# ToKe79/nuts333

Hardware: NVIDIA B200
Metric: rendered messages/sec (colour+swear+ban) (higher is better)
Workload: dtype u8

## Files before the change

### nuts333_b200/csrc/nutsb_kernels.cuh

```cuda
#pragma once
#include "nutsb_common.cuh"


struct OpsView {
    i64 n;
    const u8  *text;
    const u64 *toff;
    const u8  *kind;
    const i32 *target;
    const i32 *except_user;
    const u8  *flags;
    const i32 *gate;
    const u8  *verdict;
};

struct PopView {
    i32 n_users, n_rooms, n_rooms_tot;
    const i32 *user_room;
    const i32 *user_cls;
    const i32 *user_slot;
    const i32 *slot_user;
    const u8  *slot_cf;
    const u8  *slot_lv;
    const i32 *room_slot_off;
// ... 419 lines not shown
    u32 run_begin, run_cnt;
};

__device__ __forceinline__ uint4 nutsb_run_pack(u64 dst, u64 src, u32 len)
{
#ifdef NUTSB_EXPERIMENT_ALIGN
    dst &= ~(u64)(NUTSB_EXPERIMENT_ALIGN - 1); len = (len + NUTSB_EXPERIMENT_ALIGN - 1) & ~(u32)(NUTSB_EXPERIMENT_ALIGN - 1);
#endif
    return make_uint4((u32)dst, (u32)(dst >> 32), (u32)src, (len & 0xffffffu) | ((u32)(src >> 32) << 24));
}
#define NUTSB_RUN_MAX_LEN 0xffffffu

struct SlotInfo {
    u64 so_u;
    u64 end;
    u64 base;
    u32 b0, nb_room;
    u32 e0, e1;
    u32 room; i32 k;
    u32 cf_lv;
    u32 pad_;
};

struct SlotInfoArgs {
    PopView pop; ClassPrefix cpx;
    const u32 *room_b_off, *ev_off; const u64 *sv_pre, *stream_off;
    SlotInfo *out;
};

__global__ void __launch_bounds__(128)
k_slot_info(SlotInfoArgs A)
{
    const u32 s = blockIdx.x * blockDim.x + threadIdx.x;
    if (s >= (u32)A.pop.n_users) return;
    const i32 u = A.pop.slot_user[s];
    SlotInfo si;
    si.room = (u32)A.pop.user_room[u]; si.k = A.pop.user_cls[u];
    si.b0 = A.room_b_off[si.room]; si.nb_room = A.room_b_off[si.room + 1] - si.b0;
    si.e0 = A.ev_off[s]; si.e1 = A.ev_off[s + 1];
    si.so_u = A.stream_off[u]; si.end = A.stream_off[u + 1];
    si.base = si.so_u - A.cpx.at(si.k, si.room, si.b0) - A.sv_pre[si.e0];
    si.cf_lv = (u32)A.pop.slot_cf[s] | ((u32)A.pop.slot_lv[s] << 8);
    si.pad_ = 0;
    A.out[s] = si;
}

struct PlanArgs {
    PopView pop; Geometry geo; ClassPrefix cpx;
    const u64 *stream_off;
    const u32 *ev_off, *sv_ukey; const i32 *sv_delta; const u64 *sv_pre;
    const u32 *bl_meta;
    u64 n_cells, off_base;
    u32 has_level;
    const SlotInfo *slots;
    u32 *run_cursor;
    uint4 *runs; ItemDesc *items;
    u64 *counters;
    u32 *status;
};

template <bool FILL>
__device__ __forceinline__ u32 nutsb_plan_cell(const PlanArgs &A, u32 room, u32 t, u32 ls, u64 r_out, u32 &deliv, u32 &first)
{
    const SlotInfo si = A.slots[(u32)A.pop.room_slot_off[room] + ls];
    const u32 b0 = si.b0, nb_room = si.nb_room;
    const u32 a0 = t * NUTSB_TILE_OPS;
    const u32 nb = nb_room - a0 < NUTSB_TILE_OPS ? nb_room - a0 : NUTSB_TILE_OPS;
// ... 167 lines not shown
        const u32 l2 = (u32)idx & 15;
        const bool is_tail = idx >= 16;
        const u32 at = is_tail ? toff + l2 : l2;
        if (l2 < (is_tail ? tail : head)) dst[at] = src[at];
    }
    if (nvec == 0) return;
    dst += head; src += head;
    const u32 sm = (u32)((size_t)src & 15);
    const uint4 *sa = (const uint4 *)(src - sm);
    const u32 bsh = (sm & 3) * 8;
    switch (sm >> 2) {
    case 0:  nutsb_copy_body<0, WIDTH>(dst, sa, nvec, bsh, idx); break;
    case 1:  nutsb_copy_body<1, WIDTH>(dst, sa, nvec, bsh, idx); break;
    case 2:  nutsb_copy_body<2, WIDTH>(dst, sa, nvec, bsh, idx); break;
    default: nutsb_copy_body<3, WIDTH>(dst, sa, nvec, bsh, idx); break;
    }
}
__device__ __forceinline__ void nutsb_warp_copy(u8 *dst, const u8 *src, u32 n, int lane) { nutsb_group_copy<32>(dst, src, n, lane); }

#define NUTSB_REN_ON_WIN    3072
#define NUTSB_REN_OFF_WIN   1536
#define NUTSB_REN_ON_ROUND  (32 * 28)
#define NUTSB_REN_OFF_ROUND (32 * 8)
#define NUTSB_FL_COLOUR     0x100u

__device__ __forceinline__ u32 nutsb_keep_mask(i32 wb, i32 lo, i32 hi)
{
    i32 dl = lo - wb; dl = dl < 0 ? 0 : dl;
    i32 dh = wb + 4 - hi; dh = dh < 0 ? 0 : dh;
    const u32 a = dl >= 4 ? 0u : 0xffffffffu << (8 * dl);
    const u32 b = dh >= 4 ? 0u : 0xffffffffu >> (8 * dh);
    return a & b;
}

#define NUTSB_FLAT_META(al, n, fl) ((u32)(al) | ((u32)(n) << 2) | ((u32)(fl) << 14))

template <bool BOTH, class Sink>
__device__ __forceinline__ void nutsb_flat_render(u32 cnt, u32 meta, u64 gw, u32 nw,
                                                  u8 *w_on, u8 *w_off, const u8 *tab, int lane, Sink &sink)
{
    u32 inc = nw;
    for (int d = 1; d < 32; d <<= 1) { const u32 t = __shfl_up_sync(NUTSB_FULL, inc, d); if (lane >= d) inc += t; }
    const u32 P = inc - nw;
    const u32 W = __shfl_sync(NUTSB_FULL, inc, 31);
    u32 fill_on = 0, fill_off = 0, qcount = 0;
    u32 carry_x = 0, carry_m = 0;

    for (u32 F = 0; F < W; F += 32) {
        const bool starts = (u32)lane < cnt && P >= F && P < F + 32;
        const u32 heads = __reduce_or_sync(NUTSB_FULL, starts ? 1u << (P - F) : 0u);
        u32 q = qcount + (u32)__popc(heads & (0xffffffffu >> (31 - lane))) - 1;
        qcount += (u32)__popc(heads);
        if (q >= cnt) q = cnt - 1;
        const u32 Pq = __shfl_sync(NUTSB_FULL, P, (int)q), mq = __shfl_sync(NUTSB_FULL, meta, (int)q);
        const u32 *gwq = (const u32 *)(size_t)__shfl_sync(NUTSB_FULL, gw, (int)q);
        const u32 alq = mq & 3u, nq = (mq >> 2) & 0xfffu, flq = mq >> 14;
        const u32 endq = alq + nq;
        u32 nwq = (endq + 3) >> 2; if (!nwq) nwq = 1;
// ... 184 lines not shown
        __syncthreads();
        for (u32 r = (u32)warp / NUTSB_FAN_GROUP; r < nr; r += NUTSB_FAN_THREADS / 32 / NUTSB_FAN_GROUP) {
            const uint4 run = s_run[r];
            const u64 so = (u64)run.z | ((u64)(run.w >> 24) << 32);
            const u32 len = run.w & 0xffffffu;
            u8 *dst = A.out + (((u64)run.y << 32) | run.x);
            const u8 *src;
            if (!staged) src = A.slab + so;
            else if (so >= A.off_base) src = s_off + a_off + (u32)(so - d.off_src);
            else src = s_on + a_on + (u32)(so - d.on_src);
            nutsb_group_copy<32 * NUTSB_FAN_GROUP>(dst, src, len, tid % (32 * NUTSB_FAN_GROUP));
        }
    }
}

__global__ void __launch_bounds__(NUTSB_FAN_THREADS, NUTSB_FAN_MINBLOCKS)
k_fanout(FanoutArgs A)
{
    NUTSB_DYN_SMEM(s_dyn);
    nutsb_fanout_block(A, blockIdx.x, s_dyn);
}

struct DirectArgs {
    OpsView ops; PopView pop; ClassPrefix cpx;
    const u32 *room_b_off, *ev_off;
    const u32 *sv_ukey, *sv_op; const u64 *sv_pre;
    const u64 *stream_off;
    const u32 *ev_slot_sorted;
    const i32 *sv_delta;
    u8 *out; i64 n_ev;
    u64 *n_deliveries;
    u32 *status;
    const u8 *slab; u64 off_base;
    u32 has_level;
    const SlotInfo *slots;
    const u64 *dpre;
};

#define NUTSB_DIRECT_THREADS 256

struct DirectSink {
    u8 *out; u64 p; u32 O, osz;
    u32 cnt, done, qf;
    __device__ __forceinline__ void on(const u8 *w, u32 nbytes, int lane)
    {
        const u32 end = done + nbytes;
        while (qf < cnt) {
            const u32 Oq = __shfl_sync(NUTSB_FULL, O, (int)qf), zq = __shfl_sync(NUTSB_FULL, osz, (int)qf);
            const u64 pq = __shfl_sync(NUTSB_FULL, p, (int)qf);
            if (Oq >= end && zq) break;
            const u32 x0 = Oq > done ? Oq : done, x1 = Oq + zq < end ? Oq + zq : end;
            if (x1 > x0) {
                u8 *dst = out + pq + (x0 - Oq);
                const u8 *src = w + (x0 - done);
                const u32 len = x1 - x0;
                if (len < 192) { for (u32 i = (u32)lane; i < len; i += 32) dst[i] = src[i]; }
                else nutsb_warp_copy(dst, src, len, lane);
            }
            if (Oq + zq <= end) ++qf; else break;
        }
        done = end;
    }
    __device__ __forceinline__ void off(const u8 *, u32, int) {}
};

#define NUTSB_DIR_WARPS (NUTSB_DIRECT_THREADS / 32)
#define NUTSB_DIR_SMEM  (NUTSB_DIR_WARPS * (NUTSB_REN_ON_WIN + 64) + NUTSB_DIR_WARPS * 32 * (8 + 8 + 8) + ((NUTSB_CODETAB_BYTES + 15) & ~15))

template <bool COMPACT>
__device__ __forceinline__ void nutsb_direct_block(const DirectArgs &A, u32 blk, u32 nblk, u8 *smem)
{
    typedef u8 OnWin[NUTSB_REN_ON_WIN + 64];
    OnWin *const s_on = (OnWin *)smem;
    u64 (*const s_gw)[32] = (u64 (*)[32])(smem + NUTSB_DIR_WARPS * (NUTSB_REN_ON_WIN + 64));
    u64 (*const s_p)[32] = s_gw + NUTSB_DIR_WARPS;
    u32 (*const s_par)[32][2] = (u32 (*)[32][2])(s_p + NUTSB_DIR_WARPS);
    u8 *const s_tab = (u8 *)(s_par + NUTSB_DIR_WARPS);
    const int tid = threadIdx.x, lane = tid & 31, warp = tid >> 5;
    for (int i = tid; i < NUTSB_CODETAB_BYTES; i += NUTSB_DIRECT_THREADS) s_tab[i] = A.pop.codetab[i];
    __syncthreads();

    u64 c_cnt = 0, c_bytes = 0; u32 seam_bytes = 0;
    for (i64 ebase = ((i64)blk * (NUTSB_DIRECT_THREADS / 32) + warp) * 32; ebase < A.n_ev;
         ebase += (i64)nblk * NUTSB_DIRECT_THREADS) {
        const i64 e = ebase + lane;
        bool isw = false, seam = false, first_ev = false, last_ev = false;
        u64 p = 0, q = 0, gw = 0; u32 n = 0, al = 0, osz = 0, fl = 0;
        u64 a_start = 0, b_end = 0; const u8 *sa = nullptr, *sb = nullptr;
        if (e < A.n_ev) {
            const u32 uk = A.sv_ukey[e];
            const SlotInfo si = A.slots[A.ev_slot_sorted[e]];
            const u32 room = si.room; const i32 k = si.k;
            const u32 b0 = si.b0, cf = si.cf_lv & 0xffu;
            const u32 e0 = si.e0, e1 = si.e1;
            const u64 so_u = si.so_u, base = si.base;
            const u32 j = uk >> 2, ek = uk & 3u, skip = ek != NUTSB_EV_DIRECT;
            p = base + A.cpx.at(k, room, b0 + j) + A.sv_pre[e];
            q = base + A.cpx.at(k, room, b0 + j + skip) + A.sv_pre[e + 1];
            if (ek != NUTSB_EV_SKIP) {
                const u32 op = A.sv_op[e];
                const u64 t0 = A.ops.toff[op];
                const u8 *src = A.ops.text + t0;
                n = (u32)(A.ops.toff[op + 1] - t0);
                al = (u32)((size_t)src & 3);
                gw = (u64)(size_t)(src - al);
                nutsb_prefetch(src, n);
                fl = A.ops.flags[op] | ((cf & NUTSB_UF_COLOUR) ? NUTSB_FL_COLOUR : 0u);
                osz = (u32)(q - p);
                isw = true;
            }
            seam = !COMPACT && !A.has_level && !(cf & NUTSB_UF_FILTERED);
            if (COMPACT && isw) p = A.dpre[e];
            if (seam) {
                const bool colour = (cf & NUTSB_UF_COLOUR) != 0;
                const u64 *vp = colour ? A.cpx.vp_on : A.cpx.vp_off;
                const u8 *R = A.slab + (colour ? 0 : A.off_base);
                first_ev = (u32)e == e0; last_ev = (u32)e + 1 == e1;
                a_start = so_u; b_end = si.end;
                if (!first_ev && lane == 0) {
                    const u32 ukp = A.sv_ukey[e - 1];
                    a_start = base + A.cpx.at(k, room, b0 + (ukp >> 2) + ((ukp & 3u) != NUTSB_EV_DIRECT)) + A.sv_pre[e];
                }
                if (!last_ev && (lane == 31 || e + 1 >= A.n_ev))
                    b_end = base + A.cpx.at(k, room, b0 + (A.sv_ukey[e + 1] >> 2)) + A.sv_pre[e + 1];
                sa = R + vp[b0 + j];
                sb = R + vp[b0 + j + skip];
            }
        }
        if (!COMPACT) {
            const u64 q_prev = __shfl_up_sync(NUTSB_FULL, q, 1), p_next = __shfl_down_sync(NUTSB_FULL, p, 1);
            if (seam && !first_ev && lane > 0) a_start = q_prev;
            if (seam && !last_ev && lane < 31 && e + 1 < A.n_ev) b_end = p_next;
            u64 t0 = p & ~(u64)31; if (t0 < a_start) t0 = a_start;
            u64 h1 = (q + 31) & ~(u64)31; if (h1 > b_end) h1 = b_end;
            const u32 tlen = seam ? (u32)(p - t0) : 0u, hlen = seam && h1 > q ? (u32)(h1 - q) : 0u;
            seam_bytes += tlen + hlen;
            u8 *const stage = s_on[warp];
            const u32 lens = tlen | (hlen << 8);
            if (__any_sync(NUTSB_FULL, lens != 0)) {
#pragma unroll 8
                for (int i = 0; i < 32; ++i) {
                    const u32 l = __shfl_sync(NUTSB_FULL, lens, i);
                    const u8 *pa = (const u8 *)(size_t)__shfl_sync(NUTSB_FULL, (u64)(size_t)sa, i) - (l & 0xffu);
                    const u8 *pb = (const u8 *)(size_t)__shfl_sync(NUTSB_FULL, (u64)(size_t)sb, i);
                    u8 va = 0, vb = 0;
                    if ((u32)lane < (l & 0xffu)) va = pa[lane];
                    if ((u32)lane < (l >> 8)) vb = pb[lane];
                    stage[64 * i + lane] = va; stage[64 * i + 32 + lane] = vb;
                }
                __syncwarp();
#pragma unroll 4
                for (int i = 0; i < 32; ++i) {
                    const u32 l = __shfl_sync(NUTSB_FULL, lens, i);
                    const u64 da = __shfl_sync(NUTSB_FULL, t0, i), db = __shfl_sync(NUTSB_FULL, q, i);
                    if ((u32)lane < (l & 0xffu)) A.out[da + lane] = stage[64 * i + lane];
                    if ((u32)lane < (l >> 8)) A.out[db + lane] = stage[64 * i + 32 + lane];
                }
                __syncwarp();
            }
        }
        const u32 wmask = __ballot_sync(NUTSB_FULL, isw);
        const u32 cnt = (u32)__popc(wmask);
        if (!cnt) continue;
        if (isw) {
            const u32 r = (u32)__popc(wmask & ((1u << lane) - 1));
            s_gw[warp][r] = gw; s_p[warp][r] = p;
            s_par[warp][r][0] = NUTSB_FLAT_META(al, n, fl); s_par[warp][r][1] = osz;
        }
        __syncwarp();
        u32 nw = 0, meta = 0;
        osz = 0; gw = 0; p = 0;
        if ((u32)lane < cnt) {
            gw = s_gw[warp][lane]; p = s_p[warp][lane];
            meta = s_par[warp][lane][0]; osz = s_par[warp][lane][1];
            nw = ((meta & 3u) + ((meta >> 2) & 0xfffu) + 3) >> 2; if (!nw) nw = 1;
        }
        __syncwarp();
        u32 inc = osz;
        for (int d = 1; d < 32; d <<= 1) { const u32 t = __shfl_up_sync(NUTSB_FULL, inc, d); if (lane >= d) inc += t; }
        const u32 total = __shfl_sync(NUTSB_FULL, inc, 31);
        DirectSink sink{ A.out, p, inc - osz, osz, cnt, 0u, 0u };
        nutsb_flat_render<false>(cnt, meta, gw, nw, s_on[warp], (u8 *)nullptr, s_tab, lane, sink);
        if (lane == 0 && sink.done != total) atomicOr(A.status, NUTSB_ST_RENDER_MISMATCH);
        c_cnt += cnt; c_bytes += total;
    }
    for (int d = 16; d; d >>= 1) seam_bytes += __shfl_xor_sync(NUTSB_FULL, seam_bytes, d);
    if (lane == 0 && (c_cnt | seam_bytes)) { nutsb_add64(A.n_deliveries, c_cnt); nutsb_add64(A.n_deliveries + 1, c_bytes + seam_bytes); }
}

#ifndef NUTSB_DIR_MINBLOCKS
#define NUTSB_DIR_MINBLOCKS 5
#endif
__global__ void __launch_bounds__(NUTSB_DIRECT_THREADS, NUTSB_DIR_MINBLOCKS)
k_direct(DirectArgs A)
{
    NUTSB_DYN_SMEM(s_dyn);
    nutsb_direct_block<false>(A, blockIdx.x, gridDim.x, s_dyn);
}

__global__ void __launch_bounds__(NUTSB_DIRECT_THREADS, NUTSB_DIR_MINBLOCKS)
k_direct_compact(DirectArgs A)
{
    NUTSB_DYN_SMEM(s_dyn);
    nutsb_direct_block<true>(A, blockIdx.x, gridDim.x, s_dyn);
}

#define NUTSB_FD_SMEM (NUTSB_FAN_SMEM > NUTSB_DIR_SMEM ? NUTSB_FAN_SMEM : NUTSB_DIR_SMEM)
static_assert(NUTSB_FAN_THREADS == NUTSB_DIRECT_THREADS, "k_fanout_direct runs both bodies with one block size");
#ifndef NUTSB_FD_MINBLOCKS
#define NUTSB_FD_MINBLOCKS 5
// ... 276 lines not shown
```

### nuts333_b200/csrc/nutsb_lib.cu

```cuda
#include "nutsb_kernels.cuh"
#include "nutsb_match.cuh"
#include "nutsb_speech.cuh"

#define NUTSB_API extern "C" __attribute__((visibility("default")))

#include <algorithm>
#include <cstdio>
#include <cstdlib>
#include <cstring>
#include <deque>
#include <new>
#include <numeric>
#include <string>
#include <vector>

struct DBuf {
    void *p = nullptr; size_t cap = 0;
    template <class T> T *as() const { return (T *)p; }
};
struct HBuf {
    void *p = nullptr; size_t cap = 0;
    template <class T> T *as() const { return (T *)p; }
};

// ... 40 lines not shown
        o.target = target.empty() ? &z32 : target.data(); o.except_user = except.empty() ? &z32 : except.data();
        if (verdict) { o.gate = gate.empty() ? &z32 : gate.data(); o.verdict = verdict; }
        return o;
    }
};

enum Ev {
    EV_START,
    EV_RENDER0, EV_RENDER1,
    EV_DIRECT0, EV_DIRECT1,
    EV_FAN0, EV_FAN1,
    EV_END,
    EV_H2D0, EV_H2D1,
    EV_D2H0, EV_D2H1,
    EV_COUNT
};

struct nutsb_ctx {
    int device = 0;
    cudaStream_t stream = nullptr; bool own_stream = true;
    cudaStream_t side = nullptr; bool overlap = true;
    int side_render = 8;
    int fd_dir_per_sm = 0;
    cudaEvent_t dep[4] = {nullptr, nullptr, nullptr, nullptr};
    int sm_count = 148;
    std::string err;
    bool profiling = false; nutsb_timing tm{};
    cudaEvent_t ev[EV_COUNT] = {};

    DBuf d_codetab;
    AcDev swear, site; SetDev userban;
    bool site_file = false, user_file = false;
    std::vector<u8> ban_bytes[2];

    bool have_users = false, all_simple = true, has_clones = false;
    i32 n_clone_flag = 0, n_remote_flag = 0;
    i32 U = 0, R = 0, Rt = 1;
    std::vector<i32> user_room, user_slot, slot_user, room_slot_off;
    std::vector<u8> uflags, ulevel;
    std::vector<i32> remote_link; std::vector<u8> remote_old;
    std::vector<i32> remotes;
    std::vector<i32> clone_owner; std::vector<u8> clone_hear;
    std::vector<std::vector<i32>> room_clones;
    std::vector<std::string> room_names;
    DBuf d_user_room, d_user_slot, d_slot_user, d_room_slot_off, d_slot_cf, d_slot_lv;
    ClassSet cls[2];

    DBuf d_status, d_len_on, d_len_off, d_nrep, d_eoff, d_sums, d_scan_ticket;
    void *scan_state_seen = nullptr; size_t scan_state_cap = 0; u32 scan_epoch = 0;
    DBuf d_ek[2], d_ev_[2];
    DBuf d_hist, d_hoffs;
    DBuf d_room_ent_off, d_e_info, d_e_delta, d_e_slot, d_e_scan, d_counts, d_room_b_off;
    DBuf d_bl_op, d_bl_room, d_evk[2], d_evv[2], d_ev_ukey, d_ev_delta, d_ev_op;
    DBuf d_sv_ukey, d_sv_delta, d_sv_op, d_sv_pre, d_ev_off;
    DBuf d_vp_on, d_vp_off, d_cp;
    DBuf d_room_tile_off, d_room_cell_off, d_room_item_off, d_sizes, d_counters;
    DBuf d_runs, d_items, d_slab, d_bl_meta, d_slots;
    DBuf d_off, d_out, d_digest, d_ulen;
    DBuf d_dpre, d_dir, d_iov, d_iov_first, d_iov_cnt;
    HBuf h_small, h_off, h_out, h_dir, h_iov, h_iov_first, h_iov_cnt;
    u64 last_total = 0; bool have_streams = false;
    struct LastBatch { bool valid = false; OpsView ops{}; ClassPrefix cpx{}; bool has_level = false; u64 off_base = 0; u32 *sv_slot = nullptr; } last;
    DBuf d_room_users, d_room_users_off, d_dg;

    DBuf s_text, s_toff, s_kind, s_target, s_except, s_flags, s_gate, s_verdict, s_v8;

    bool have_names = false; bool ban_swearing = false;
    std::vector<u8> names, sflags; std::vector<u64> name_off;
    std::vector<std::string> lits;
    DBuf d_names, d_name_off, d_sflags, d_lit, d_lit_off;
    DBuf d_sp_len, d_sp_off, d_sp_text, d_sp_kind, d_sp_target, d_sp_except, d_sp_flags, d_sp_gate, d_sp_verdict;
    DBuf s_verb, s_speaker, s_body, s_boff;
    i32 shard = -1, g_U = 0; bool have_g_names = false;
    DBuf d_g_user_shard, d_g_user_local, d_g_has_room, d_g_names, d_g_name_off, d_g_sflags, d_sp_keep, d_sp_sel;

    HostOps q;
    std::vector<u8> q_sw_text; std::vector<u64> q_sw_off{0};
    std::vector<u8> q_sw_verdict;

    struct RevBuf { char buf[NUTSB_REVIEW_LINES][NUTSB_REVIEW_LEN + 2]; int line; };
// ... 282 lines not shown
    case NUTSB_E_RANGE: return "value out of range";
    case NUTSB_E_STATE: return "call order";
    }
    return "unknown";
}
NUTSB_API const char *nutsb_last_error(const nutsb_ctx *c) { return c ? c->err.c_str() : ""; }

NUTSB_API void nutsb_destroy(nutsb_ctx *c)
{
    if (!c) return;
    cudaSetDevice(c->device);
    if (c->stream) cudaStreamSynchronize(c->stream);
    DBuf *all[] = { &c->d_codetab, &c->swear.trans, &c->swear.clsmap, &c->swear.tr16, &c->swear.cls2, &c->site.trans, &c->site.clsmap, &c->site.tr16, &c->site.cls2,
        &c->userban.slot_off, &c->userban.slot_len, &c->userban.pool,
        &c->d_user_room, &c->d_user_slot, &c->d_slot_user, &c->d_room_slot_off, &c->d_slot_cf, &c->d_slot_lv,
        &c->cls[0].d_user_cls, &c->cls[0].d_room_cls_off, &c->cls[0].d_cls_flags, &c->cls[0].d_cls_level,
        &c->cls[1].d_user_cls, &c->cls[1].d_room_cls_off, &c->cls[1].d_cls_flags, &c->cls[1].d_cls_level,
        &c->d_status, &c->d_len_on, &c->d_len_off, &c->d_nrep, &c->d_eoff, &c->d_sums, &c->d_scan_ticket, &c->d_ek[0], &c->d_ek[1],
        &c->d_ev_[0], &c->d_ev_[1], &c->d_hist, &c->d_hoffs, &c->d_room_ent_off, &c->d_e_info, &c->d_e_delta,
        &c->d_e_slot, &c->d_e_scan, &c->d_counts, &c->d_room_b_off, &c->d_bl_op, &c->d_bl_room, &c->d_evk[0],
        &c->d_evk[1], &c->d_evv[0], &c->d_evv[1], &c->d_ev_ukey, &c->d_ev_delta, &c->d_ev_op, &c->d_sv_ukey,
        &c->d_sv_delta, &c->d_sv_op, &c->d_sv_pre, &c->d_ev_off, &c->d_vp_on, &c->d_vp_off, &c->d_cp,
        &c->d_room_tile_off, &c->d_room_cell_off, &c->d_room_item_off, &c->d_sizes, &c->d_counters,
        &c->d_runs, &c->d_slots, &c->d_items, &c->d_slab, &c->d_bl_meta, &c->d_off, &c->d_out, &c->d_digest, &c->d_ulen,
        &c->d_dpre, &c->d_dir, &c->d_iov, &c->d_iov_first, &c->d_iov_cnt, &c->d_room_users, &c->d_room_users_off, &c->d_dg,
        &c->s_text, &c->s_toff, &c->s_kind, &c->s_target, &c->s_except, &c->s_flags, &c->s_gate, &c->s_verdict, &c->s_v8,
        &c->d_names, &c->d_name_off, &c->d_sflags, &c->d_lit, &c->d_lit_off, &c->d_sp_len, &c->d_sp_off, &c->d_sp_text,
        &c->d_sp_kind, &c->d_sp_target, &c->d_sp_except, &c->d_sp_flags, &c->d_sp_gate, &c->d_sp_verdict,
        &c->s_verb, &c->s_speaker, &c->s_body, &c->s_boff,
        &c->d_g_user_shard, &c->d_g_user_local, &c->d_g_has_room, &c->d_g_names, &c->d_g_name_off, &c->d_g_sflags, &c->d_sp_keep, &c->d_sp_sel,
        &c->d_rec_key, &c->d_rec_line, &c->d_rec_k[0], &c->d_rec_k[1], &c->d_rec_v[0], &c->d_rec_v[1], &c->d_rec_cnt, &c->d_rec_seg,
        &c->d_rec_lens, &c->d_rec_bytes, &c->d_rec_off, &c->d_rec_out };
    for (DBuf *b : all) release(*b);
    release(c->h_small); release(c->h_off); release(c->h_out);
    release(c->h_dir); release(c->h_iov); release(c->h_iov_first); release(c->h_iov_cnt); release(c->h_rec);
    for (auto &e : c->ev) if (e) cudaEventDestroy(e);
    for (auto &e : c->dep) if (e) cudaEventDestroy(e);
    if (c->side) { cudaStreamSynchronize(c->side); cudaStreamDestroy(c->side); }
    if (c->own_stream && c->stream) cudaStreamDestroy(c->stream);
    delete c;
}

static int set_swear_impl(nutsb_ctx *c, const char *const *words)
{
    std::vector<std::string> pats;
    for (size_t i = 0; words && words[i] && words[i][0] != '*'; ++i) pats.emplace_back(words[i]);
    AcHost h; build_ac(pats, true, h);
// ... 303 lines not shown
                   u64 slab, u64 fan_in, u64 fan_out, u64 render_in)
{
    c->last_total = total; c->have_streams = bytes != nullptr;
    c->tm.slab_bytes = slab; c->tm.fanout_bytes_in = fan_in; c->tm.fanout_bytes_out = fan_out; c->tm.render_bytes_in = render_in;
    out->n_users = c->U; out->total_bytes = total; out->n_deliveries = deliveries;
    out->off = c->d_off.as<u64>(); out->bytes = bytes; out->on_device = 1;
}

static int write_iov_tail(nutsb_ctx *c, const Planned &p, nutsb_streams *out, IovReq *iv)
{
    const i32 U = c->U; const Sizes &sz = p.sz;
    cudaStream_t st = c->stream;
    u32 *h32 = c->h_small.as<u32>(); u64 *h64 = c->h_small.as<u64>();
    *iv = IovReq{ true, p.off_base + p.slab_off, sz.direct_bytes, 2ull * sz.n_events + (u64)U };
    TRY(ensure(c, c->d_dir, sz.direct_bytes + 64));
    TRY(ensure(c, c->d_iov, (size_t)iv->n_iov * sizeof(IovEnt)));
    TRY(ensure(c, c->d_iov_first, (size_t)U * 8)); TRY(ensure(c, c->d_iov_cnt, (size_t)U * 4));
    TRY(ensure_host(c, c->h_dir, (size_t)sz.direct_bytes + 64));
    TRY(ensure_host(c, c->h_iov, (size_t)iv->n_iov * sizeof(IovEnt)));
    TRY(ensure_host(c, c->h_iov_first, ((size_t)U + 1) * 8)); TRY(ensure_host(c, c->h_iov_cnt, ((size_t)U + 1) * 4));
    TRY(ensure_host(c, c->h_off, ((size_t)U + 1) * 8));
    TRY(ev_record(c, EV_DIRECT0, st));
    if (sz.n_events > 0) {
        DirectArgs da{ p.ops, p.pop, p.cpx, c->d_room_b_off.as<u32>(), c->d_ev_off.as<u32>(), c->d_sv_ukey.as<u32>(), c->d_sv_op.as<u32>(),
                       c->d_sv_pre.as<u64>(), c->d_off.as<u64>(), p.sv_slot, c->d_sv_delta.as<i32>(), c->d_dir.as<u8>(), (i64)sz.n_events, p.counters,
                       c->d_status.as<u32>(), c->d_slab.as<u8>(), p.off_base, 0u, c->d_slots.as<SlotInfo>(), c->d_dpre.as<u64>() };
        NUTSB_LAUNCH_SMEM(cdiv(sz.n_events, NUTSB_DIRECT_THREADS), NUTSB_DIRECT_THREADS, NUTSB_DIR_SMEM, st, k_direct_compact, da); CKL();
        c->tm.launches++;
    }
    TRY(ev_record(c, EV_DIRECT1, st)); TRY(ev_record(c, EV_FAN0, st));
    IovArgs ia{ p.pop, c->d_slots.as<SlotInfo>(), c->d_vp_on.as<u64>(), c->d_vp_off.as<u64>(), c->d_sv_ukey.as<u32>(), p.sv_slot,
                c->d_dpre.as<u64>(), sz.n_events, (u64)(size_t)c->h_out.p, (u64)(size_t)c->h_dir.p, p.off_base,
                c->d_iov.as<IovEnt>(), c->d_iov_first.as<u64>(), c->d_iov_cnt.as<u32>(), p.counters };
    NUTSB_LAUNCH(cdiv(std::max<u64>(sz.n_events, (u64)U), 256), 256, st, k_iov, ia); CKL();
    c->tm.launches++;
    TRY(ev_record(c, EV_FAN1, st)); TRY(ev_record(c, EV_END, st));
    if (sz.direct_bytes) CK(cudaMemcpyAsync(c->h_dir.p, c->d_dir.p, (size_t)sz.direct_bytes, cudaMemcpyDeviceToHost, st));
    CK(cudaMemcpyAsync(c->h_iov.p, c->d_iov.p, (size_t)iv->n_iov * sizeof(IovEnt), cudaMemcpyDeviceToHost, st));
    CK(cudaMemcpyAsync(c->h_iov_first.p, c->d_iov_first.p, (size_t)U * 8, cudaMemcpyDeviceToHost, st));
    CK(cudaMemcpyAsync(c->h_iov_cnt.p, c->d_iov_cnt.p, (size_t)U * 4, cudaMemcpyDeviceToHost, st));
    CK(cudaMemcpyAsync(c->h_off.p, c->d_off.p, ((size_t)U + 1) * 8, cudaMemcpyDeviceToHost, st));
    CK(cudaMemcpyAsync(h64 + 8, p.counters, 24, cudaMemcpyDeviceToHost, st));
    CK(cudaMemcpyAsync(h32 + 4, c->d_status.p, 4, cudaMemcpyDeviceToHost, st));
    if (p.par) CK(cudaStreamWaitEvent(st, c->dep[1], 0));
    TRY(ev_record(c, EV_D2H1, st));
    CK(cudaStreamSynchronize(st));
    TRY(status_to_error(c, h32[4]));
    if (c->profiling) {
        TRY(ev_elapsed(c, &c->tm.plan_ms, EV_START, EV_DIRECT0));
        TRY(ev_elapsed(c, &c->tm.render_ms, EV_RENDER0, EV_RENDER1));
        TRY(ev_elapsed(c, &c->tm.fanout_ms, EV_FAN0, EV_FAN1));
        TRY(ev_elapsed(c, &c->tm.direct_ms, EV_DIRECT0, EV_DIRECT1));
        TRY(ev_elapsed(c, &c->tm.total_ms, EV_START, EV_END));
        TRY(ev_elapsed(c, &c->tm.d2h_ms, EV_END, EV_D2H1));
    }
    finish(c, out, nullptr, sz.total_bytes, h64[8], p.slab_on + p.slab_off, 0, 0, h64[10]);
    return NUTSB_OK;
}

static int write_streams_tail(nutsb_ctx *c, const Planned &p, nutsb_streams *out)
{
    const Sizes &sz = p.sz;
    cudaStream_t st = c->stream, sd = p.sd;
    u32 *h32 = c->h_small.as<u32>(); u64 *h64 = c->h_small.as<u64>();
    TRY(ensure(c, c->d_out, sz.total_bytes + 64));
    Geometry geo{ c->d_room_b_off.as<u32>(), c->d_room_tile_off.as<u32>(), c->d_room_cell_off.as<u64>(), c->d_room_item_off.as<u32>() };

    const bool fan = sz.cells > 0 && sz.items > 0;
    const bool fused = p.par && fan && sz.n_events > 0;
    DirectArgs da{ p.ops, p.pop, p.cpx, c->d_room_b_off.as<u32>(), c->d_ev_off.as<u32>(), c->d_sv_ukey.as<u32>(), c->d_sv_op.as<u32>(),
                   c->d_sv_pre.as<u64>(), c->d_off.as<u64>(), p.sv_slot, c->d_sv_delta.as<i32>(), c->d_out.as<u8>(), (i64)sz.n_events, p.counters,
                   c->d_status.as<u32>(), c->d_slab.as<u8>(), p.off_base, p.has_level ? 1u : 0u, c->d_slots.as<SlotInfo>(), nullptr };
    u32 n_dir = cdiv(sz.n_events, NUTSB_DIRECT_THREADS);
    if (fused && c->fd_dir_per_sm > 0) n_dir = std::min(n_dir, (u32)(c->sm_count * c->fd_dir_per_sm));
    TRY(ev_record(c, EV_DIRECT0, sd));
    if (sz.n_events > 0 && !fused) {
        if (p.par) { CK(cudaEventRecord(c->dep[2], st)); CK(cudaStreamWaitEvent(sd, c->dep[2], 0)); }
        NUTSB_LAUNCH_SMEM(n_dir, NUTSB_DIRECT_THREADS, NUTSB_DIR_SMEM, sd, k_direct, da); CKL();
        c->tm.launches++;
    }
    TRY(ev_record(c, EV_DIRECT1, sd));
    if (p.par) CK(cudaEventRecord(c->dep[3], sd));

    if (fan) {
        TRY(ensure(c, c->d_items, (size_t)sz.items * sizeof(ItemDesc)));
        u32 *cursor = p.counts + 4;
        CK(cudaMemsetAsync(cursor, 0, 4, st));
        PlanArgs pa{ p.pop, geo, p.cpx, c->d_off.as<u64>(), c->d_ev_off.as<u32>(), c->d_sv_ukey.as<u32>(), c->d_sv_delta.as<i32>(),
                     c->d_sv_pre.as<u64>(), c->d_bl_meta.as<u32>(), (u64)sz.cells, p.off_base, p.has_level ? 1u : 0u,
                     c->d_slots.as<SlotInfo>(), cursor, nullptr, c->d_items.as<ItemDesc>(), p.counters, c->d_status.as<u32>() };
        u64 n_runs = sz.cells + sz.n_events;
        if (!p.alias) {
            NUTSB_LAUNCH(sz.items, NUTSB_UCHUNK, st, k_plan<false>, pa); CKL();
            CK(cudaMemcpyAsync(h32 + 6, cursor, 4, cudaMemcpyDeviceToHost, st));
            CK(cudaMemsetAsync(cursor, 0, 4, st));
            CK(cudaStreamSynchronize(st));
            n_runs = h32[6];
            c->tm.launches++;
        }
        if (n_runs >= 0xfffffff0ull) return fail(c, NUTSB_E_RANGE, "more than 2^32 copy runs in one batch%s");
        TRY(ensure(c, c->d_runs, (n_runs + 1) * sizeof(uint4)));
        pa.runs = c->d_runs.as<uint4>();
        NUTSB_LAUNCH(sz.items, NUTSB_UCHUNK, st, k_plan<true>, pa); CKL();
        c->tm.launches++;
    }

// ... 159 lines not shown
        RenderArgs ra{ ops, c->d_codetab.as<u8>(), c->d_bl_op.as<u32>(), c->d_vp_on.as<u64>(), c->d_vp_off.as<u64>(), counts,
                       c->d_slab.as<u8>(), off_base, counters, c->d_status.as<u32>() };
        u32 grid = cdiv(E, NUTSB_REN_OPS * (NUTSB_REN_THREADS / 32));
        if (par) grid = std::min(grid, (u32)(c->sm_count * c->side_render));
        NUTSB_LAUNCH(grid, NUTSB_REN_THREADS, sd, k_render, ra); CKL();
        c->tm.launches++;
    }
    TRY(ev_record(c, EV_RENDER1, sd));
    if (compact && off_base + slab_off) CK(cudaMemcpyAsync(c->h_out.p, c->d_slab.p, (size_t)(off_base + slab_off), cudaMemcpyDeviceToHost, sd));
    if (par) CK(cudaEventRecord(c->dep[1], sd));

    u32 *sv_slot = nullptr, *perm = nullptr;
    TRY(radix_sort(c, c->d_evk, c->d_evv, (i64)E, counts + 1, bits_for((u64)std::max(U, 1)), &sv_slot, &perm));
    TRY(ensure(c, c->d_sv_ukey, E * 4 + 16)); TRY(ensure(c, c->d_sv_delta, E * 4 + 16)); TRY(ensure(c, c->d_sv_op, E * 4 + 16));
    TRY(ensure(c, c->d_sv_pre, (E + 2) * 8)); TRY(ensure(c, c->d_ev_off, ((size_t)U + 2) * 4));
    NUTSB_LAUNCH(cdiv(E + 1, 256), 256, st, k_ev_gather, perm, counts + 1, c->d_ev_ukey.as<u32>(), c->d_ev_delta.as<i32>(),
                 c->d_ev_op.as<u32>(), c->d_sv_ukey.as<u32>(), c->d_sv_delta.as<i32>(), c->d_sv_op.as<u32>(), sv_slot, (u32)U, c->d_ev_off.as<u32>()); CKL();
    TRY(run_scan(c, InI32{c->d_sv_delta.as<i32>()}, OutU64{c->d_sv_pre.as<u64>()}, (i64)E, counts + 1));
    c->tm.launches += 1;

    UserLenIn uli{ cpx, pop, c->d_room_b_off.as<u32>(), c->d_ev_off.as<u32>(), c->d_sv_pre.as<u64>() };
    TRY(run_scan(c, uli, OutU64{c->d_off.as<u64>()}, (i64)U, nullptr));
    TRY(ensure(c, c->d_slots, ((size_t)U + 1) * sizeof(SlotInfo)));
    if (U > 0) {
        SlotInfoArgs sa{ pop, cpx, c->d_room_b_off.as<u32>(), c->d_ev_off.as<u32>(), c->d_sv_pre.as<u64>(), c->d_off.as<u64>(), c->d_slots.as<SlotInfo>() };
        NUTSB_LAUNCH(cdiv((u64)U, 128), 128, st, k_slot_info, sa); CKL();
        c->tm.launches++;
    }
    if (compact) {
        TRY(ensure(c, c->d_dpre, (E + 2) * 8));
        TRY(run_scan(c, InDirectLen{ c->d_sv_ukey.as<u32>(), sv_slot, c->d_sv_delta.as<i32>(), c->d_slots.as<SlotInfo>(),
                                     c->d_vp_on.as<u64>(), c->d_vp_off.as<u64>() }, OutU64{c->d_dpre.as<u64>()}, (i64)E, counts + 1));
    }
    TRY(ensure(c, c->d_room_tile_off, ((size_t)Rt + 2) * 4)); TRY(ensure(c, c->d_room_cell_off, ((size_t)Rt + 2) * 8));
    TRY(ensure(c, c->d_room_item_off, ((size_t)Rt + 2) * 4));
    Sizes *hs = (Sizes *)(c->h_small.as<u8>() + 256);
    NUTSB_LAUNCH(1, NUTSB_SCAN_THREADS, st, k_geometry, pop, c->d_room_b_off.as<u32>(), c->d_off.as<u64>(), counts,
                 c->d_vp_on.as<u64>(), c->d_vp_off.as<u64>(),
                 c->d_room_tile_off.as<u32>(), c->d_room_cell_off.as<u64>(), c->d_room_item_off.as<u32>(), hs,
                 compact ? c->d_dpre.as<u64>() : (const u64 *)nullptr); CKL();
    c->tm.launches++;
    CK(cudaStreamSynchronize(st));
    const Planned p{ ops, pop, cpx, *hs, sv_slot, counts, counters, off_base, slab_on, slab_off, has_level, alias, par, sd };
    if (p.sz.slab_on != slab_on || p.sz.slab_off != slab_off) return fail(c, NUTSB_E_CUDA, "internal: slab size mismatch%s");
    return compact ? write_iov_tail(c, p, out, iv) : write_streams_tail(c, p, out);
}

static int check_ops(nutsb_ctx *c, const nutsb_ops *o)
{
    if (!c || !o || o->n_ops < 0) return fail(c, NUTSB_E_INVAL, "null argument or negative n_ops%s");
    if (o->n_ops >= 0xfffffff0ll) return fail(c, NUTSB_E_RANGE, "more than 2^32 ops in one batch%s");
// ... 975 lines not shown
```

Baseline: 34.93 billion.

## Precompute per-event direct-render records in slot-info kernel on side stream

Moves the per-event address, metadata and seam computation out of the direct render kernel into k_slot_info, which now writes a packed DirRec per event. The direct kernel then loads one record per lane instead of chasing slot, prefix and ops arrays, and the slot-info kernel can run on the side stream overlapped with the main stream. This adds an extra E-sized buffer write and read, plus event dependencies. Seam neighbour bounds are now computed per event from global memory rather than by warp shuffles.

```diff
diff --git a/nuts333_b200/csrc/nutsb_kernels.cuh b/nuts333_b200/csrc/nutsb_kernels.cuh
--- a/nuts333_b200/csrc/nutsb_kernels.cuh
+++ b/nuts333_b200/csrc/nutsb_kernels.cuh
@@ -465,27 +465,88 @@
     u32 pad_;
 };
 
+#define NUTSB_FL_COLOUR     0x100u
+#define NUTSB_FLAT_META(al, n, fl) ((u32)(al) | ((u32)(n) << 2) | ((u32)(fl) << 14))
+
+struct __align__(16) DirRec {
+    u64 p, q;
+    u64 gw;
+    u64 src_tail, src_head;
+    u32 meta;
+    u32 lens;
+};
+#define NUTSB_DR_DIRECT 0x10000u
+
 struct SlotInfoArgs {
-    PopView pop; ClassPrefix cpx;
+    PopView pop; ClassPrefix cpx; OpsView ops;
     const u32 *room_b_off, *ev_off; const u64 *sv_pre, *stream_off;
-    SlotInfo *out;
-};
+    const u32 *sv_slot, *sv_ukey, *sv_op, *n_ev;
+    u64 off_base; u32 has_level;
+    SlotInfo *out; DirRec *rec;
+};
+
+__device__ __forceinline__ void nutsb_dir_rec(const SlotInfoArgs &A, u32 e)
+{
+    const u32 s = A.sv_slot[e];
+    const i32 u = A.pop.slot_user[s];
+    const u32 room = (u32)A.pop.user_room[u]; const i32 k = A.pop.user_cls[u];
+    const u32 b0 = A.room_b_off[room], e0 = A.ev_off[s], e1 = A.ev_off[s + 1];
+    const u32 cf = A.pop.slot_cf[s];
+    const u64 so_u = A.stream_off[u];
+    const u64 base = so_u - A.cpx.at(k, room, b0) - A.sv_pre[e0];
+    const u32 uk = A.sv_ukey[e], j = uk >> 2, ek = uk & 3u, skip = ek != NUTSB_EV_DIRECT;
+    DirRec r;
+    r.p = base + A.cpx.at(k, room, b0 + j) + A.sv_pre[e];
+    r.q = base + A.cpx.at(k, room, b0 + j + skip) + A.sv_pre[e + 1];
+    r.gw = 0; r.meta = 0; r.lens = 0; r.src_tail = 0; r.src_head = 0;
+    if (ek != NUTSB_EV_SKIP) {
+        const u32 op = A.sv_op[e];
+        const u64 t0 = A.ops.toff[op];
+        const u8 *src = A.ops.text + t0;
+        const u32 al = (u32)((size_t)src & 3);
+        r.gw = (u64)(size_t)(src - al);
+        r.meta = NUTSB_FLAT_META(al, (u32)(A.ops.toff[op + 1] - t0), A.ops.flags[op] | ((cf & NUTSB_UF_COLOUR) ? NUTSB_FL_COLOUR : 0u));
+        r.lens = NUTSB_DR_DIRECT;
+    }
+    if (!A.has_level && !(cf & NUTSB_UF_FILTERED)) {
+        u64 a_start = so_u, b_end = A.stream_off[u + 1];
+        if (e != e0) {
+            const u32 ukp = A.sv_ukey[e - 1];
+            a_start = base + A.cpx.at(k, room, b0 + (ukp >> 2) + ((ukp & 3u) != NUTSB_EV_DIRECT)) + A.sv_pre[e];
+        }
+        if (e + 1 != e1) b_end = base + A.cpx.at(k, room, b0 + (A.sv_ukey[e + 1] >> 2)) + A.sv_pre[e + 1];
+        u64 t0 = r.p & ~(u64)31; if (t0 < a_start) t0 = a_start;
+        u64 h1 = (r.q + 31) & ~(u64)31; if (h1 > b_end) h1 = b_end;
+        const u32 tlen = (u32)(r.p - t0), hlen = h1 > r.q ? (u32)(h1 - r.q) : 0u;
+        const bool colour = (cf & NUTSB_UF_COLOUR) != 0;
+        const u64 *vp = colour ? A.cpx.vp_on : A.cpx.vp_off;
+        const u64 R = colour ? 0 : A.off_base;
+        r.src_tail = R + vp[b0 + j] - tlen;
+        r.src_head = R + vp[b0 + j + skip];
+        r.lens |= tlen | (hlen << 8);
+    }
+    A.rec[e] = r;
+}
 
 __global__ void __launch_bounds__(128)
 k_slot_info(SlotInfoArgs A)
 {
-    const u32 s = blockIdx.x * blockDim.x + threadIdx.x;
-    if (s >= (u32)A.pop.n_users) return;
-    const i32 u = A.pop.slot_user[s];
-    SlotInfo si;
-    si.room = (u32)A.pop.user_room[u]; si.k = A.pop.user_cls[u];
-    si.b0 = A.room_b_off[si.room]; si.nb_room = A.room_b_off[si.room + 1] - si.b0;
-    si.e0 = A.ev_off[s]; si.e1 = A.ev_off[s + 1];
-    si.so_u = A.stream_off[u]; si.end = A.stream_off[u + 1];
-    si.base = si.so_u - A.cpx.at(si.k, si.room, si.b0) - A.sv_pre[si.e0];
-    si.cf_lv = (u32)A.pop.slot_cf[s] | ((u32)A.pop.slot_lv[s] << 8);
-    si.pad_ = 0;
-    A.out[s] = si;
+    const u32 t = blockIdx.x * blockDim.x + threadIdx.x;
+    if (t < (u32)A.pop.n_users) {
+        const u32 s = t;
+        const i32 u = A.pop.slot_user[s];
+        SlotInfo si;
+        si.room = (u32)A.pop.user_room[u]; si.k = A.pop.user_cls[u];
+        si.b0 = A.room_b_off[si.room]; si.nb_room = A.room_b_off[si.room + 1] - si.b0;
+        si.e0 = A.ev_off[s]; si.e1 = A.ev_off[s + 1];
+        si.so_u = A.stream_off[u]; si.end = A.stream_off[u + 1];
+        si.base = si.so_u - A.cpx.at(si.k, si.room, si.b0) - A.sv_pre[si.e0];
+        si.cf_lv = (u32)A.pop.slot_cf[s] | ((u32)A.pop.slot_lv[s] << 8);
+        si.pad_ = 0;
+        A.out[s] = si;
+    }
+    const u32 n_ev = *A.n_ev;
+    for (u32 e = t; e < n_ev; e += gridDim.x * blockDim.x) nutsb_dir_rec(A, e);
 }
 
 struct PlanArgs {
@@ -699,7 +760,6 @@
 #define NUTSB_REN_OFF_WIN   1536
 #define NUTSB_REN_ON_ROUND  (32 * 28)
 #define NUTSB_REN_OFF_ROUND (32 * 8)
-#define NUTSB_FL_COLOUR     0x100u
 
 __device__ __forceinline__ u32 nutsb_keep_mask(i32 wb, i32 lo, i32 hi)
 {
@@ -710,7 +770,6 @@
     return a & b;
 }
 
-#define NUTSB_FLAT_META(al, n, fl) ((u32)(al) | ((u32)(n) << 2) | ((u32)(fl) << 14))
 
 template <bool BOTH, class Sink>
 __device__ __forceinline__ void nutsb_flat_render(u32 cnt, u32 meta, u64 gw, u32 nw,
@@ -941,18 +1000,12 @@
 }
 
 struct DirectArgs {
-    OpsView ops; PopView pop; ClassPrefix cpx;
-    const u32 *room_b_off, *ev_off;
-    const u32 *sv_ukey, *sv_op; const u64 *sv_pre;
-    const u64 *stream_off;
-    const u32 *ev_slot_sorted;
-    const i32 *sv_delta;
+    const DirRec *rec;
+    const u8 *codetab;
     u8 *out; i64 n_ev;
     u64 *n_deliveries;
     u32 *status;
-    const u8 *slab; u64 off_base;
-    u32 has_level;
-    const SlotInfo *slots;
+    const u8 *slab;
     const u64 *dpre;
 };
 
@@ -996,72 +1049,35 @@
     u32 (*const s_par)[32][2] = (u32 (*)[32][2])(s_p + NUTSB_DIR_WARPS);
     u8 *const s_tab = (u8 *)(s_par + NUTSB_DIR_WARPS);
     const int tid = threadIdx.x, lane = tid & 31, warp = tid >> 5;
-    for (int i = tid; i < NUTSB_CODETAB_BYTES; i += NUTSB_DIRECT_THREADS) s_tab[i] = A.pop.codetab[i];
+    for (int i = tid; i < NUTSB_CODETAB_BYTES; i += NUTSB_DIRECT_THREADS) s_tab[i] = A.codetab[i];
     __syncthreads();
 
-    u64 c_cnt = 0, c_bytes = 0; u32 seam_bytes = 0;
+    u32 c_cnt = 0; u64 c_bytes = 0;
     for (i64 ebase = ((i64)blk * (NUTSB_DIRECT_THREADS / 32) + warp) * 32; ebase < A.n_ev;
          ebase += (i64)nblk * NUTSB_DIRECT_THREADS) {
         const i64 e = ebase + lane;
-        bool isw = false, seam = false, first_ev = false, last_ev = false;
-        u64 p = 0, q = 0, gw = 0; u32 n = 0, al = 0, osz = 0, fl = 0;
-        u64 a_start = 0, b_end = 0; const u8 *sa = nullptr, *sb = nullptr;
+        bool isw = false;
+        u64 p = 0, q = 0, gw = 0, st = 0, sh = 0; u32 meta = 0, osz = 0, lens = 0;
         if (e < A.n_ev) {
-            const u32 uk = A.sv_ukey[e];
-            const SlotInfo si = A.slots[A.ev_slot_sorted[e]];
-            const u32 room = si.room; const i32 k = si.k;
-            const u32 b0 = si.b0, cf = si.cf_lv & 0xffu;
-            const u32 e0 = si.e0, e1 = si.e1;
-            const u64 so_u = si.so_u, base = si.base;
-            const u32 j = uk >> 2, ek = uk & 3u, skip = ek != NUTSB_EV_DIRECT;
-            p = base + A.cpx.at(k, room, b0 + j) + A.sv_pre[e];
-            q = base + A.cpx.at(k, room, b0 + j + skip) + A.sv_pre[e + 1];
-            if (ek != NUTSB_EV_SKIP) {
-                const u32 op = A.sv_op[e];
-                const u64 t0 = A.ops.toff[op];
-                const u8 *src = A.ops.text + t0;
-                n = (u32)(A.ops.toff[op + 1] - t0);
-                al = (u32)((size_t)src & 3);
-                gw = (u64)(size_t)(src - al);
-                nutsb_prefetch(src, n);
-                fl = A.ops.flags[op] | ((cf & NUTSB_UF_COLOUR) ? NUTSB_FL_COLOUR : 0u);
+            const DirRec r = A.rec[e];
+            p = r.p; q = r.q; gw = r.gw; meta = r.meta;
+            isw = (r.lens & NUTSB_DR_DIRECT) != 0;
+            if (isw) {
+                nutsb_prefetch((const u8 *)(size_t)gw + (meta & 3u), (meta >> 2) & 0xfffu);
                 osz = (u32)(q - p);
-                isw = true;
+                if (COMPACT) p = A.dpre[e];
             }
-            seam = !COMPACT && !A.has_level && !(cf & NUTSB_UF_FILTERED);
-            if (COMPACT && isw) p = A.dpre[e];
-            if (seam) {
-                const bool colour = (cf & NUTSB_UF_COLOUR) != 0;
-                const u64 *vp = colour ? A.cpx.vp_on : A.cpx.vp_off;
-                const u8 *R = A.slab + (colour ? 0 : A.off_base);
-                first_ev = (u32)e == e0; last_ev = (u32)e + 1 == e1;
-                a_start = so_u; b_end = si.end;
-                if (!first_ev && lane == 0) {
-                    const u32 ukp = A.sv_ukey[e - 1];
-                    a_start = base + A.cpx.at(k, room, b0 + (ukp >> 2) + ((ukp & 3u) != NUTSB_EV_DIRECT)) + A.sv_pre[e];
-                }
-                if (!last_ev && (lane == 31 || e + 1 >= A.n_ev))
-                    b_end = base + A.cpx.at(k, room, b0 + (A.sv_ukey[e + 1] >> 2)) + A.sv_pre[e + 1];
-                sa = R + vp[b0 + j];
-                sb = R + vp[b0 + j + skip];
-            }
+            if (!COMPACT) { lens = r.lens & 0xffffu; st = r.src_tail; sh = r.src_head; }
         }
         if (!COMPACT) {
-            const u64 q_prev = __shfl_up_sync(NUTSB_FULL, q, 1), p_next = __shfl_down_sync(NUTSB_FULL, p, 1);
-            if (seam && !first_ev && lane > 0) a_start = q_prev;
-            if (seam && !last_ev && lane < 31 && e + 1 < A.n_ev) b_end = p_next;
-            u64 t0 = p & ~(u64)31; if (t0 < a_start) t0 = a_start;
-            u64 h1 = (q + 31) & ~(u64)31; if (h1 > b_end) h1 = b_end;
-            const u32 tlen = seam ? (u32)(p - t0) : 0u, hlen = seam && h1 > q ? (u32)(h1 - q) : 0u;
-            seam_bytes += tlen + hlen;
+            c_bytes += (lens & 0xffu) + (lens >> 8);
             u8 *const stage = s_on[warp];
-            const u32 lens = tlen | (hlen << 8);
             if (__any_sync(NUTSB_FULL, lens != 0)) {
 #pragma unroll 8
                 for (int i = 0; i < 32; ++i) {
                     const u32 l = __shfl_sync(NUTSB_FULL, lens, i);
-                    const u8 *pa = (const u8 *)(size_t)__shfl_sync(NUTSB_FULL, (u64)(size_t)sa, i) - (l & 0xffu);
-                    const u8 *pb = (const u8 *)(size_t)__shfl_sync(NUTSB_FULL, (u64)(size_t)sb, i);
+                    const u8 *pa = A.slab + __shfl_sync(NUTSB_FULL, st, i);
+                    const u8 *pb = A.slab + __shfl_sync(NUTSB_FULL, sh, i);
                     u8 va = 0, vb = 0;
                     if ((u32)lane < (l & 0xffu)) va = pa[lane];
                     if ((u32)lane < (l >> 8)) vb = pb[lane];
@@ -1071,7 +1087,7 @@
 #pragma unroll 4
                 for (int i = 0; i < 32; ++i) {
                     const u32 l = __shfl_sync(NUTSB_FULL, lens, i);
-                    const u64 da = __shfl_sync(NUTSB_FULL, t0, i), db = __shfl_sync(NUTSB_FULL, q, i);
+                    const u64 da = __shfl_sync(NUTSB_FULL, p, i) - (l & 0xffu), db = __shfl_sync(NUTSB_FULL, q, i);
                     if ((u32)lane < (l & 0xffu)) A.out[da + lane] = stage[64 * i + lane];
                     if ((u32)lane < (l >> 8)) A.out[db + lane] = stage[64 * i + 32 + lane];
                 }
@@ -1084,11 +1100,11 @@
         if (isw) {
             const u32 r = (u32)__popc(wmask & ((1u << lane) - 1));
             s_gw[warp][r] = gw; s_p[warp][r] = p;
-            s_par[warp][r][0] = NUTSB_FLAT_META(al, n, fl); s_par[warp][r][1] = osz;
+            s_par[warp][r][0] = meta; s_par[warp][r][1] = osz;
         }
         __syncwarp();
-        u32 nw = 0, meta = 0;
-        osz = 0; gw = 0; p = 0;
+        u32 nw = 0;
+        meta = 0; osz = 0; gw = 0; p = 0;
         if ((u32)lane < cnt) {
             gw = s_gw[warp][lane]; p = s_p[warp][lane];
             meta = s_par[warp][lane][0]; osz = s_par[warp][lane][1];
@@ -1101,10 +1117,10 @@
         DirectSink sink{ A.out, p, inc - osz, osz, cnt, 0u, 0u };
         nutsb_flat_render<false>(cnt, meta, gw, nw, s_on[warp], (u8 *)nullptr, s_tab, lane, sink);
         if (lane == 0 && sink.done != total) atomicOr(A.status, NUTSB_ST_RENDER_MISMATCH);
-        c_cnt += cnt; c_bytes += total;
-    }
-    for (int d = 16; d; d >>= 1) seam_bytes += __shfl_xor_sync(NUTSB_FULL, seam_bytes, d);
-    if (lane == 0 && (c_cnt | seam_bytes)) { nutsb_add64(A.n_deliveries, c_cnt); nutsb_add64(A.n_deliveries + 1, c_bytes + seam_bytes); }
+        if (lane == 0) { c_cnt += cnt; c_bytes += total; }
+    }
+    for (int d = 16; d; d >>= 1) c_bytes += __shfl_xor_sync(NUTSB_FULL, c_bytes, d);
+    if (lane == 0 && (c_cnt | c_bytes)) { nutsb_add64(A.n_deliveries, c_cnt); nutsb_add64(A.n_deliveries + 1, c_bytes); }
 }
 
 #ifndef NUTSB_DIR_MINBLOCKS
diff --git a/nuts333_b200/csrc/nutsb_lib.cu b/nuts333_b200/csrc/nutsb_lib.cu
--- a/nuts333_b200/csrc/nutsb_lib.cu
+++ b/nuts333_b200/csrc/nutsb_lib.cu
@@ -86,7 +86,7 @@
     cudaStream_t side = nullptr; bool overlap = true;
     int side_render = 8;
     int fd_dir_per_sm = 0;
-    cudaEvent_t dep[4] = {nullptr, nullptr, nullptr, nullptr};
+    cudaEvent_t dep[6] = {nullptr, nullptr, nullptr, nullptr, nullptr, nullptr};
     int sm_count = 148;
     std::string err;
     bool profiling = false; nutsb_timing tm{};
@@ -119,7 +119,7 @@
     DBuf d_sv_ukey, d_sv_delta, d_sv_op, d_sv_pre, d_ev_off;
     DBuf d_vp_on, d_vp_off, d_cp;
     DBuf d_room_tile_off, d_room_cell_off, d_room_item_off, d_sizes, d_counters;
-    DBuf d_runs, d_items, d_slab, d_bl_meta, d_slots;
+    DBuf d_runs, d_items, d_slab, d_bl_meta, d_slots, d_dirrec;
     DBuf d_off, d_out, d_digest, d_ulen;
     DBuf d_dpre, d_dir, d_iov, d_iov_first, d_iov_cnt;
     HBuf h_small, h_off, h_out, h_dir, h_iov, h_iov_first, h_iov_cnt;
@@ -448,7 +448,7 @@
         &c->d_evk[1], &c->d_evv[0], &c->d_evv[1], &c->d_ev_ukey, &c->d_ev_delta, &c->d_ev_op, &c->d_sv_ukey,
         &c->d_sv_delta, &c->d_sv_op, &c->d_sv_pre, &c->d_ev_off, &c->d_vp_on, &c->d_vp_off, &c->d_cp,
         &c->d_room_tile_off, &c->d_room_cell_off, &c->d_room_item_off, &c->d_sizes, &c->d_counters,
-        &c->d_runs, &c->d_slots, &c->d_items, &c->d_slab, &c->d_bl_meta, &c->d_off, &c->d_out, &c->d_digest, &c->d_ulen,
+        &c->d_runs, &c->d_slots, &c->d_dirrec, &c->d_items, &c->d_slab, &c->d_bl_meta, &c->d_off, &c->d_out, &c->d_digest, &c->d_ulen,
         &c->d_dpre, &c->d_dir, &c->d_iov, &c->d_iov_first, &c->d_iov_cnt, &c->d_room_users, &c->d_room_users_off, &c->d_dg,
         &c->s_text, &c->s_toff, &c->s_kind, &c->s_target, &c->s_except, &c->s_flags, &c->s_gate, &c->s_verdict, &c->s_v8,
         &c->d_names, &c->d_name_off, &c->d_sflags, &c->d_lit, &c->d_lit_off, &c->d_sp_len, &c->d_sp_off, &c->d_sp_text,
@@ -798,9 +798,8 @@
     TRY(ensure_host(c, c->h_off, ((size_t)U + 1) * 8));
     TRY(ev_record(c, EV_DIRECT0, st));
     if (sz.n_events > 0) {
-        DirectArgs da{ p.ops, p.pop, p.cpx, c->d_room_b_off.as<u32>(), c->d_ev_off.as<u32>(), c->d_sv_ukey.as<u32>(), c->d_sv_op.as<u32>(),
-                       c->d_sv_pre.as<u64>(), c->d_off.as<u64>(), p.sv_slot, c->d_sv_delta.as<i32>(), c->d_dir.as<u8>(), (i64)sz.n_events, p.counters,
-                       c->d_status.as<u32>(), c->d_slab.as<u8>(), p.off_base, 0u, c->d_slots.as<SlotInfo>(), c->d_dpre.as<u64>() };
+        DirectArgs da{ c->d_dirrec.as<DirRec>(), p.pop.codetab, c->d_dir.as<u8>(), (i64)sz.n_events, p.counters, c->d_status.as<u32>(),
+                       c->d_slab.as<u8>(), c->d_dpre.as<u64>() };
         NUTSB_LAUNCH_SMEM(cdiv(sz.n_events, NUTSB_DIRECT_THREADS), NUTSB_DIRECT_THREADS, NUTSB_DIR_SMEM, st, k_direct_compact, da); CKL();
         c->tm.launches++;
     }
@@ -844,9 +843,8 @@
 
     const bool fan = sz.cells > 0 && sz.items > 0;
     const bool fused = p.par && fan && sz.n_events > 0;
-    DirectArgs da{ p.ops, p.pop, p.cpx, c->d_room_b_off.as<u32>(), c->d_ev_off.as<u32>(), c->d_sv_ukey.as<u32>(), c->d_sv_op.as<u32>(),
-                   c->d_sv_pre.as<u64>(), c->d_off.as<u64>(), p.sv_slot, c->d_sv_delta.as<i32>(), c->d_out.as<u8>(), (i64)sz.n_events, p.counters,
-                   c->d_status.as<u32>(), c->d_slab.as<u8>(), p.off_base, p.has_level ? 1u : 0u, c->d_slots.as<SlotInfo>(), nullptr };
+    DirectArgs da{ c->d_dirrec.as<DirRec>(), p.pop.codetab, c->d_out.as<u8>(), (i64)sz.n_events, p.counters, c->d_status.as<u32>(),
+                   c->d_slab.as<u8>(), nullptr };
     u32 n_dir = cdiv(sz.n_events, NUTSB_DIRECT_THREADS);
     if (fused && c->fd_dir_per_sm > 0) n_dir = std::min(n_dir, (u32)(c->sm_count * c->fd_dir_per_sm));
     TRY(ev_record(c, EV_DIRECT0, sd));
@@ -858,6 +856,7 @@
     TRY(ev_record(c, EV_DIRECT1, sd));
     if (p.par) CK(cudaEventRecord(c->dep[3], sd));
 
+    if (p.par) CK(cudaStreamWaitEvent(st, c->dep[5], 0));
     if (fan) {
         TRY(ensure(c, c->d_items, (size_t)sz.items * sizeof(ItemDesc)));
         u32 *cursor = p.counts + 4;
@@ -1063,11 +1062,27 @@
     UserLenIn uli{ cpx, pop, c->d_room_b_off.as<u32>(), c->d_ev_off.as<u32>(), c->d_sv_pre.as<u64>() };
     TRY(run_scan(c, uli, OutU64{c->d_off.as<u64>()}, (i64)U, nullptr));
     TRY(ensure(c, c->d_slots, ((size_t)U + 1) * sizeof(SlotInfo)));
+    TRY(ensure(c, c->d_dirrec, (size_t)E * sizeof(DirRec)));
+    const bool slot_side = par && !compact;
+#ifdef NUTSB_EXP_SLOT_MAIN
+    const bool slot_side_x = false;
+#else
+    const bool slot_side_x = slot_side;
+#endif
+    cudaStream_t ss = slot_side_x ? sd : st;
+    if (slot_side) { CK(cudaEventRecord(c->dep[4], st)); if (slot_side_x) CK(cudaStreamWaitEvent(sd, c->dep[4], 0)); }
     if (U > 0) {
-        SlotInfoArgs sa{ pop, cpx, c->d_room_b_off.as<u32>(), c->d_ev_off.as<u32>(), c->d_sv_pre.as<u64>(), c->d_off.as<u64>(), c->d_slots.as<SlotInfo>() };
-        NUTSB_LAUNCH(cdiv((u64)U, 128), 128, st, k_slot_info, sa); CKL();
+        SlotInfoArgs sa{ pop, cpx, ops, c->d_room_b_off.as<u32>(), c->d_ev_off.as<u32>(), c->d_sv_pre.as<u64>(), c->d_off.as<u64>(),
+                         sv_slot, c->d_sv_ukey.as<u32>(), c->d_sv_op.as<u32>(), counts + 1, off_base, has_level ? 1u : 0u,
+                         c->d_slots.as<SlotInfo>(), c->d_dirrec.as<DirRec>() };
+#ifndef NUTSB_EXP_SLOT_CAP
+#define NUTSB_EXP_SLOT_CAP 16
+#endif
+        const u32 grid = std::max(cdiv((u64)U, 128), NUTSB_EXP_SLOT_CAP ? std::min(cdiv(E, 128), (u32)c->sm_count * NUTSB_EXP_SLOT_CAP) : cdiv(E, 128));
+        NUTSB_LAUNCH(grid, 128, ss, k_slot_info, sa); CKL();
         c->tm.launches++;
     }
+    if (slot_side) CK(cudaEventRecord(c->dep[5], ss));
     if (compact) {
         TRY(ensure(c, c->d_dpre, (E + 2) * 8));
         TRY(run_scan(c, InDirectLen{ c->d_sv_ukey.as<u32>(), sv_slot, c->d_sv_delta.as<i32>(), c->d_slots.as<SlotInfo>(),
```

Result: no change. 35.03 billion (median of 6 runs) (+0.3%).
